# revdotcom/reverb

Measured on AMD Instinct MI355X. Metric: RTFx (audio-sec/wall-sec) Reverb-ASR attention_rescoring, higher is better.
Workload: dtype bf16

## Files before the change

reverb_amd/csrc/engine.h:

```cpp
#pragma once
#include <condition_variable>
#include <functional>
#include <map>
#include <mutex>
#include <string>
#include <thread>
#include <vector>

#include "../../include/rvb.h"
#include "kernels.h"
#include "search.h"

namespace rvb {

struct HostTensor {
  std::vector<float> data;
  std::vector<int64_t> shape;
  size_t numel() const { size_t n = 1; for (auto s : shape) n *= (size_t)s; return n; }
};

struct DevBuf {
  void* p = nullptr;
  size_t bytes = 0;
  int ensure(size_t n);
// ... 93 lines not shown
  unsigned long long gen_ = 0;
  bool stop_ = false;
};

struct HypRef { int chunk, idx, len, row0; };

struct TrieBatch {
  int R = 0, P = 0, max_chunk_rows = 0;
  std::vector<int32_t> tok, pos;
  std::vector<int32_t> path;
  std::vector<int32_t> hq_start, hq_len, hq_pos0, hkv_start, hkv_len;
  std::vector<int32_t> crow_start, crow_len;
  std::vector<int32_t> tgt_ptr, tgt;
  std::vector<int32_t> pair_slot;
  std::vector<int32_t> work;
};

struct CtcAligner {
  std::vector<VitSeq> seq;
  std::vector<int32_t> h_tokens, h_rows;
  int max_S = 0, blank = 0;
  size_t alpha_floats = 0, bp_bytes = 0;
  int64_t total_frames = 0;
  DevBuf d_tokens, d_rows, d_seqs, d_alpha, d_bp, d_states, d_score;
  int plan(const char* who, const int32_t* tokens, const int32_t* tok_lens, int n_seq, const std::vector<std::vector<int32_t>>& seq_rows,
           int V, int blank_id);
  int begin(hipStream_t s);
  bool touches(int r0, int nrows) const;
  int advance(hipStream_t s, const float* lp, int ld, int r0, int nrows);
  int finish(hipStream_t s, int32_t* states , float* score );
  void release();
};

}

struct rvb_engine {
  rvb_model_cfg cfg;
  int device = 0;
  int dtype = 0;
  bool fp8 = false;
  int f8_state = 0;
  std::vector<rvb::F8Scales> f8;
  std::vector<unsigned> f8_groups;
  rvb::DevBuf d_amax;
  bool f8_conv2 = false;
  float f8_x1 = 0.f;
  rvb::DevBuf d_f8sat;
  hipStream_t stream = nullptr;
  bool finalized = false;

  std::map<std::string, rvb::HostTensor> host;

  rvb::DevBuf cmvn_mean, cmvn_istd, conv1_w, conv1_b;
  rvb::Linear conv2, embed_out, ctc;
  rvb::LNorm enc_after;
  std::vector<rvb::EncLayer> enc;
  rvb::Decoder dec_l, dec_r;
  rvb::DevBuf pe_f32;
  int pe_rows = 0;
  rvb::DevBuf fb_window, fb_twiddle, fb_melw, fb_lo, fb_hi;
  rvb::DevBuf stage;

  rvb::DevBuf pcm, feats;
  rvb::DevBuf pcm_next;
  hipStream_t copy_stream = nullptr;
  hipEvent_t pcm_ready = nullptr, pcm_free = nullptr;
  bool pcm_pending = false;
  int64_t n_samples_next = 0;
  rvb::DevBuf wave_f32, rs_kernel;
  rvb::DevBuf wave_in;
  bool pcm_is_float = false;
  int dec_chunk = 0, dec_left = -1;
  int64_t n_samples = 0, n_frames = 0, feat_rows = 0;

  int B = 0, T0 = 0, T1 = 0, F1 = 0, T2 = 0, F2 = 0, beam = 0;
  std::vector<int32_t> in_lens, enc_lens;
  rvb::DevBuf d_feats_in, X1, X2, x, xn, y, h, ao, dconv, enc_out, logits, topv, topi;
  rvb::DevBuf d_enc_lens, d_seq_start, d_seq_len, d_aux_i32;
  float* h_topv = nullptr;
  int32_t* h_topi = nullptr;
  size_t h_top_cap = 0;
  struct Slice { int c0, nb; hipEvent_t ev; bool done; };
  std::vector<Slice> slices;
  std::vector<hipEvent_t> slice_event_pool;
  int xattn_max_rows = 0;
  const int* cur_lens = nullptr;
  std::vector<rvb::PrefixResult> nbest;
  std::vector<rvb::RescoreResult> rescored;
  std::vector<rvb::TrieBatch> trie_l;
  rvb::HostPool pool;
  std::vector<rvb::JointResult> joint;
  std::vector<rvb::DevBuf> jkv;
  rvb::DevBuf jlogp, jpair_row, jpair_tok, jpair_out;
  int64_t joint_rows = 0, joint_steps = 0;
  float last_blank_penalty = 0.f;
  std::vector<std::vector<int>> attn_tokens;
  std::vector<float> attn_scores;
  rvb::DevBuf atopv, atopi;
  std::vector<rvb::DevBuf> kcache, vcache, kcache2, vcache2, memkv;
  rvb::DevBuf dx, dxn, dy, dh, dqkv, dq, dao, kvmem, d_tok, d_pos, d_tgt, d_logp;
  rvb::DevBuf d_hq_start, d_hq_len, d_hkv_start, d_hkv_len;
  rvb::DevBuf d_hq_pos0, d_hpath_start, d_hpath_len, d_path, d_work, d_tgt_ptr;
  int64_t rescore_rows = 0, rescore_pairs = 0;

  struct StreamState {
    bool active = false;
    int offset = 0;
    int cache_len = 0;
    std::vector<rvb::DevBuf> kv, kv2;
    int cnn_rows = 0;
    std::vector<rvb::DevBuf> cnn, cnn2;
  } stream_st;
  rvb::DevBuf d_stream_i32;

  rvb::CtcAligner aligner;
  rvb::DevBuf align_lp, align_tv, align_ti, align_row, align_col, align_out;

  void* comm = nullptr;
  int comm_world = 1, comm_rank = 0;
  rvb::DevBuf comm_send, comm_recv;

  int profiling = 0;
  std::map<std::string, rvb::ProfEntry> prof;
  struct Pending { hipEvent_t a, b; std::string name; };
  std::vector<Pending> pending;
  std::vector<hipEvent_t> event_pool;
};
```

reverb_amd/csrc/engine.hip:

```cpp
#include "engine.h"

#include <algorithm>
#include <atomic>
#include <condition_variable>
#include <functional>
#include <mutex>
#include <chrono>
#include <cmath>
#include <cstdlib>
#include <cstring>
#include <thread>

namespace rvb {

static thread_local std::string g_err;
void set_error(const std::string& msg) { g_err = msg; }
const char* last_error() { return g_err.c_str(); }

int DevBuf::ensure(size_t n) {
  if (n <= bytes && p) return OK;
  if (p) { (void)hipFree(p); p = nullptr; bytes = 0; }
  if (n == 0) n = 16;
  hipError_t err = hipMalloc(&p, n);
  if (err != hipSuccess) {
    p = nullptr;
    (void)hipGetLastError();
    set_error("hipMalloc of " + std::to_string(n) + " bytes failed: " + hipGetErrorString(err));
    return E_NOMEM;
  }
  bytes = n;
  return OK;
}
void DevBuf::release() { if (p) (void)hipFree(p); p = nullptr; bytes = 0; }

#define RVB_TRY(expr) do { int _r = (expr); if (_r != OK) return _r; } while (0)

struct Scope {
  rvb_engine* e; hipEvent_t a = nullptr, b = nullptr; std::string name;
  Scope(rvb_engine* e_, const char* n, double flops = 0.0, double bytes = 0.0) : e(e_), name(n) {
    auto& pe = e->prof[name];
    pe.launches += 1; pe.flops += flops; pe.bytes += bytes;
    if (e->profiling == 0 || (e->profiling == 2 && name != "gemm" && name != "gemm_fp8")) return;
    auto get = [&]() { hipEvent_t ev; if (!e->event_pool.empty()) { ev = e->event_pool.back(); e->event_pool.pop_back(); } else (void)hipEventCreate(&ev); return ev; };
    a = get(); b = get();
    (void)hipEventRecord(a, e->stream);
  }
  ~Scope() {
    if (!a) return;
    (void)hipEventRecord(b, e->stream);
    e->pending.push_back({a, b, name});
  }
};
static void drain_prof(rvb_engine* e) {
  if (e->pending.empty()) return;
  (void)hipStreamSynchronize(e->stream);
  for (auto& p : e->pending) {
    float ms = 0.f;
    (void)hipEventElapsedTime(&ms, p.a, p.b);
    e->prof[p.name].ms += ms;
    e->event_pool.push_back(p.a); e->event_pool.push_back(p.b);
  }
  e->pending.clear();
}

static int upload_f32(rvb_engine* e, DevBuf& dst, const float* src, size_t n) {
  RVB_TRY(dst.ensure(n * 4));
  RVB_HIP_CHECK(hipMemcpyAsync(dst.p, src, n * 4, hipMemcpyHostToDevice, e->stream));
  return OK;
}
static int upload_i32(rvb_engine* e, DevBuf& dst, const int32_t* src, size_t n) {
  RVB_TRY(dst.ensure(n * 4 + 16));
  if (n) RVB_HIP_CHECK(hipMemcpyAsync(dst.p, src, n * 4, hipMemcpyHostToDevice, e->stream));
  return OK;
}
static int pack_T(rvb_engine* e, DevBuf& dst, const float* src, size_t n) {
  RVB_TRY(dst.ensure(n * dt_size(e->dtype)));
  if (e->dtype == DT_F32) {
    RVB_HIP_CHECK(hipMemcpyAsync(dst.p, src, n * 4, hipMemcpyHostToDevice, e->stream));
    return OK;
  }
  RVB_TRY(e->stage.ensure(n * 4));
  RVB_HIP_CHECK(hipMemcpyAsync(e->stage.p, src, n * 4, hipMemcpyHostToDevice, e->stream));
  return convert_f32(e->stream, e->dtype, e->stage.as<float>(), dst.p, n);
}
static int pack_linear(rvb_engine* e, Linear& L, const float* w, const float* b, int out, int in, bool f8 = false) {
  L.out = out; L.in = in;
  RVB_TRY(pack_T(e, L.w, w, (size_t)out * in));
  if (b) RVB_TRY(upload_f32(e, L.b, b, out)); else L.b.release();
  if (f8 && e->fp8 && in % 128 == 0) {
    std::vector<uint8_t> q((size_t)out * in);
    std::vector<float> sc(out);
    for (int n = 0; n < out; ++n) {
      const float* row = w + (size_t)n * in;
      float am = 0.f;
      for (int k = 0; k < in; ++k) am = std::max(am, std::fabs(row[k]));
      const float sn = am > 0.f ? am / 448.f : 1.f;
      sc[n] = sn;
      const float inv = 1.f / sn;
      for (int k = 0; k < in; ++k) q[(size_t)n * in + k] = f32_to_fp8_host(row[k] * inv);
    }
    RVB_TRY(L.w8.ensure(q.size()));
    RVB_HIP_CHECK(hipMemcpyAsync(L.w8.p, q.data(), q.size(), hipMemcpyHostToDevice, e->stream));
    RVB_TRY(upload_f32(e, L.wscale, sc.data(), out));
    RVB_HIP_CHECK(hipStreamSynchronize(e->stream));
  }
  return OK;
}

static const HostTensor* find(rvb_engine* e, const std::string& name) {
  auto it = e->host.find(name);
  return it == e->host.end() ? nullptr : &it->second;
}
static int need(rvb_engine* e, const std::string& name, size_t numel, const HostTensor** out) {
  const HostTensor* t = find(e, name);
  if (!t) { set_error("missing tensor: " + name); return E_STATE; }
  if (t->numel() != numel) {
    set_error("tensor " + name + " has " + std::to_string(t->numel()) + " elements, expected " + std::to_string(numel));
    return E_ARG;
  }
  *out = t;
  return OK;
}
static int pack_named_linear(rvb_engine* e, Linear& L, const std::string& p, int out, int in, bool bias = true, bool f8 = false) {
  const HostTensor *w, *b = nullptr;
  RVB_TRY(need(e, p + ".weight", (size_t)out * in, &w));
  if (bias) RVB_TRY(need(e, p + ".bias", out, &b));
  return pack_linear(e, L, w->data.data(), b ? b->data.data() : nullptr, out, in, f8);
}
static int pack_norm(rvb_engine* e, LNorm& n, const std::string& p, int d, float eps) {
  const HostTensor *g, *b;
  RVB_TRY(need(e, p + ".weight", d, &g));
  RVB_TRY(need(e, p + ".bias", d, &b));
  n.eps = eps;
  RVB_TRY(upload_f32(e, n.g, g->data.data(), d));
  return upload_f32(e, n.b, b->data.data(), d);
}
static int pack_concat(rvb_engine* e, Linear& L, const std::vector<std::string>& names, int out_each, int in, bool f8 = false) {
  std::vector<float> w((size_t)names.size() * out_each * in), b((size_t)names.size() * out_each);
  for (size_t i = 0; i < names.size(); ++i) {
    const HostTensor *tw, *tb;
    RVB_TRY(need(e, names[i] + ".weight", (size_t)out_each * in, &tw));
    RVB_TRY(need(e, names[i] + ".bias", out_each, &tb));
    memcpy(w.data() + i * (size_t)out_each * in, tw->data.data(), (size_t)out_each * in * 4);
    memcpy(b.data() + i * (size_t)out_each, tb->data.data(), (size_t)out_each * 4);
  }
  int r = pack_linear(e, L, w.data(), b.data(), (int)names.size() * out_each, in, f8);
// ... 423 lines not shown
    RVB_TRY(run_norm(e, x, L.n_conv, e->xn.p, false, M, d, NORM_LN, 0, nullptr, nullptr, nullptr, sc8.in_pw1, 0.f, false, satp(3)));
    RVB_TRY(run_gemm8(e, e->xn.p, d, L.pw1, e->h.p, 2 * d, M, sc8.in_pw1, 0));
  } else {
    RVB_TRY(run_norm(e, x, L.n_conv, e->xn.p, false, M, d));
    RVB_TRY(note(3, e->xn.p, (size_t)M * d));
    {
      const char* ge = lab_env("RVB_GLU_FUSE");
      const int glu_on = ge ? atoi(ge) : GLU_FUSE_DEFAULT;
      GemmArgs t;
      memset(&t, 0, sizeof(t));
      t.A = e->xn.p; t.W = L.pw1_glu.w.p; t.bias = L.pw1_glu.b.as<float>(); t.C = e->h.p; t.M = M; t.N = 2 * d; t.K = d; t.lda = d; t.ldw = d;
      t.ldc = d; t.alpha = 1.f; t.act = ACT_GLU;
      glu_fused = glu_on && li < 0 && L.pw1_glu.w.p != nullptr && !cal && gemm_glu_supported(e->dtype, t);
      if (glu_fused) {
        Scope sc(e, "gemm", 2.0 * M * (double)t.N * t.K, gemm_alg_bytes(e, t));
        RVB_TRY(gemm(e->stream, e->dtype, t));
      } else {
        RVB_TRY(run_gemm(e, e->xn.p, d, L.pw1, e->h.p, 2 * d, M, false));
      }
    }
  }
  {
    GluDwArgs g;
    g.gated = glu_fused ? 1 : 0;
    g.G = e->h.p; g.pw1_bias = L.pw1.b.as<float>(); g.dw_w = L.dw_w.as<float>(); g.dw_b = L.dw_b.as<float>();
    g.lens = e->cur_lens; g.out = e->dconv.as<float>(); g.B = B; g.T = T; g.d = d; g.K = e->cfg.cnn_kernel;
    g.causal = e->cfg.cnn_causal ? 1 : 0;
    g.out_bf16 = e->dtype == DT_BF16 ? 1 : 0;
    const int lorder = g.K - 1;
    const bool cached = li >= 0 && g.causal && lorder > 0;
    if (cached) { g.hist = e->stream_st.cnn[li].p; g.hist_rows = e->stream_st.cnn_rows; }
    {
      Scope sc(e, "glu_dwconv");
      RVB_TRY(glu_dwconv(e->stream, e->dtype, g));
    }
    if (cached) {
      auto& st = e->stream_st;
      const size_t es = dt_size(e->dtype), rb = (size_t)2 * d * es;
      if (M >= lorder) {
        RVB_HIP_CHECK(hipMemcpyAsync(st.cnn[li].p, (const char*)e->h.p + (size_t)(M - lorder) * rb, (size_t)lorder * rb,
                                     hipMemcpyDeviceToDevice, e->stream));
      } else {
        RVB_HIP_CHECK(hipMemcpyAsync(st.cnn2[li].p, (const char*)st.cnn[li].p + (size_t)M * rb, (size_t)(lorder - M) * rb,
                                     hipMemcpyDeviceToDevice, e->stream));
        RVB_HIP_CHECK(hipMemcpyAsync((char*)st.cnn2[li].p + (size_t)(lorder - M) * rb, e->h.p, (size_t)M * rb,
                                     hipMemcpyDeviceToDevice, e->stream));
        std::swap(st.cnn[li], st.cnn2[li]);
      }
    }
  }
  const int cmode = e->cfg.cnn_norm == 0 ? NORM_LN : NORM_AFFINE;
  const bool dw16 = e->dtype == DT_BF16;
  if (f8_pw2) {
    RVB_TRY(run_norm(e, e->dconv.as<float>(), L.n_cnn, e->xn.p, false, M, d, cmode, 1, nullptr, nullptr, nullptr, sc8.in_pw2, 0.f, dw16, satp(4)));
    RVB_TRY(run_gemm8(e, e->xn.p, d, L.pw2, x, d, M, sc8.in_pw2, 1, 1.f, 1.f, ACT_NONE, x, d));
  } else {
    RVB_TRY(run_norm(e, e->dconv.as<float>(), L.n_cnn, e->xn.p, false, M, d, cmode, 1, nullptr, nullptr, nullptr, 0.f, 0.f, dw16));
    RVB_TRY(note(4, e->xn.p, (size_t)M * d));
    RVB_TRY(run_gemm(e, e->xn.p, d, L.pw2, x, d, M, true, 1.f, ACT_NONE, x, d));
  }
  if (f8_ff) {
    RVB_TRY(run_norm(e, x, L.n_ff, e->xn.p, false, M, d, NORM_LN, 0, nullptr, nullptr, nullptr, sc8.in_ff1, 0.f, false, satp(5)));
    RVB_TRY(run_gemm8(e, e->xn.p, d, L.ff1, e->h.p, ff, M, sc8.in_ff1, 2, sc8.h_ff, 1.f, ACT_SILU, nullptr, 0, satp(6)));
    RVB_TRY(run_gemm8(e, e->h.p, ff, L.ff2, x, d, M, sc8.h_ff, 1, 1.f, 0.5f, ACT_NONE, x, d));
  } else {
    RVB_TRY(run_norm(e, x, L.n_ff, e->xn.p, false, M, d));
    const void* ffin = e->xn.p;
    if (L.is_lsl) {
      RVB_TRY(run_gemm(e, e->xn.p, d, L.lsl, e->y.p, d, M, false));
      ffin = e->y.p;
    } else {
      RVB_TRY(note(5, e->xn.p, (size_t)M * d));
    }
    RVB_TRY(run_gemm(e, ffin, d, L.ff1, e->h.p, ff, M, false, 1.f, ACT_SILU));
    if (!L.is_lsl) RVB_TRY(note(6, e->h.p, (size_t)M * ff));
    RVB_TRY(run_gemm(e, e->h.p, ff, L.ff2, x, d, M, true, 0.5f, ACT_NONE, x, d));
  }
  RVB_TRY(run_norm(e, x, L.n_final, x, true, M, d, NORM_LN, 0, L.is_lsl ? e->y.p : nullptr, &next, next_out, 0.f, f8 ? next8 : 0.f, false,
                   nullptr, (f8 && next8 > 0.f && e->d_f8sat.p) ? e->d_f8sat.as<unsigned>() + (size_t)(lidx + 1) * 8 : nullptr));
  return OK;
}

static const int LOGIT_SLAB = 8192;

static int wait_slices(rvb_engine* e, int i);

static int encode_impl(rvb_engine* e, const float* feats, int64_t first_chunk, const int32_t* lens, int B, int T0,
                       int beam, float blank_penalty) {
  const rvb_model_cfg& c = e->cfg;
  if (!e->finalized) { set_error("rvb_encode before rvb_finalize"); return E_STATE; }
  if (B <= 0 || B > c.max_chunks || T0 < 7 || T0 > c.chunk_frames) {
    set_error("rvb_encode: need 1 <= B <= max_chunks and 7 <= T0 <= chunk_frames"); return E_ARG;
  }
  if (beam < 1 || beam > 64 || beam > c.vocab) { set_error("rvb_encode: beam must be in [1,64]"); return E_ARG; }
  RVB_HIP_CHECK(hipSetDevice(e->device));
  RVB_TRY(wait_slices(e, -1));
  e->stream_st.active = false;
  const int d = c.d_model, F0 = c.input_dim, V = c.vocab;
  const int T1 = (T0 - 3) / 2 + 1, F1 = (F0 - 3) / 2 + 1, T2 = (T1 - 3) / 2 + 1, F2 = (F1 - 3) / 2 + 1;
  const int M = B * T2;
  const size_t es = dt_size(e->dtype);
  e->B = B; e->T0 = T0; e->T1 = T1; e->F1 = F1; e->T2 = T2; e->F2 = F2; e->beam = beam;
  e->dec_l.kv_ready = e->dec_r.kv_ready = false;
  e->last_blank_penalty = blank_penalty;
  e->in_lens.assign(lens, lens + B);
  e->enc_lens.resize(B);
  std::vector<int32_t> starts(B), qlens(B, T2);
  for (int b = 0; b < B; ++b) {
    if (lens[b] < 0 || lens[b] > T0) { set_error("rvb_encode: lens out of range"); return E_ARG; }
    e->enc_lens[b] = lens[b] > 6 ? (lens[b] - 7) / 4 + 1 : 0;
    starts[b] = b * T2;
  }
  e->nbest.clear(); e->trie_l.clear(); e->rescored.clear();
  RVB_TRY(upload_i32(e, e->d_enc_lens, e->enc_lens.data(), B));
  RVB_TRY(upload_i32(e, e->d_seq_start, starts.data(), B));
  RVB_TRY(upload_i32(e, e->d_seq_len, qlens.data(), B));

  const float* d_feats;
  if (feats) {
    RVB_TRY(upload_f32(e, e->d_feats_in, feats, (size_t)B * T0 * F0));
    d_feats = e->d_feats_in.as<float>();
  } else {
    if (!e->feats.p || (first_chunk + B) * (int64_t)T0 > e->feat_rows) {
      set_error("rvb_encode: device features missing or too short (call rvb_fbank first)"); return E_STATE;
    }
    d_feats = e->feats.as<float>() + (size_t)first_chunk * T0 * F0;
  }
  int SB = B >= 16 ? (B * 7 + 9) / 10 : B;
  if (B >= 64) SB = B - 32;
  if (const char* ov = lab_env("RVB_SLICE0")) { const int v = atoi(ov); if (v > 0 && v <= B) SB = v; }
  const int Ms = SB * T2;
  RVB_TRY(e->X1.ensure((size_t)SB * T1 * F1 * d * es));
  RVB_TRY(e->X2.ensure((size_t)SB * T2 * F2 * d * es));
  RVB_TRY(e->x.ensure((size_t)Ms * d * 4));
  RVB_TRY(e->xn.ensure((size_t)Ms * d * es));
  RVB_TRY(e->y.ensure((size_t)Ms * d * es));
  RVB_TRY(e->ao.ensure((size_t)Ms * d * es));
  RVB_TRY(e->dconv.ensure((size_t)Ms * d * 4));
  RVB_TRY(e->enc_out.ensure((size_t)M * d * es));
  RVB_TRY(e->h.ensure((size_t)Ms * std::max(c.ffn_dim, 3 * d) * es));
  const int Vld = (V + 3) & ~3;
  RVB_TRY(e->logits.ensure((size_t)LOGIT_SLAB * Vld * 4));
  RVB_TRY(e->topv.ensure((size_t)M * beam * 4));
  RVB_TRY(e->topi.ensure((size_t)M * beam * 4));
  if (e->h_top_cap < (size_t)M * beam) {
    if (e->h_topv) (void)hipHostFree(e->h_topv);
    if (e->h_topi) (void)hipHostFree(e->h_topi);
    e->h_topv = nullptr; e->h_topi = nullptr; e->h_top_cap = 0;
    RVB_HIP_CHECK(hipHostMalloc((void**)&e->h_topv, (size_t)M * beam * 4, hipHostMallocDefault));
    RVB_HIP_CHECK(hipHostMalloc((void**)&e->h_topi, (size_t)M * beam * 4, hipHostMallocDefault));
    e->h_top_cap = (size_t)M * beam;
  }
  e->slices.clear();
  if (e->fp8 && e->f8_state == 0) {
    RVB_TRY(e->d_amax.ensure((e->enc.size() + 1) * 8 * 4));
    RVB_HIP_CHECK(hipMemsetAsync(e->d_amax.p, 0, (e->enc.size() + 1) * 8 * 4, e->stream));
    RVB_TRY(reset_f8sat(e));
    e->f8_state = 1;
  }
  for (int c0 = 0; c0 < B; c0 += SB) {
    const int nb = std::min(SB, B - c0);
    const int m = nb * T2;
    const int row0 = c0 * T2;
    e->cur_lens = e->d_enc_lens.as<int>() + c0;
    const bool f8c2 = e->fp8 && e->f8_state == 2 && e->f8_conv2 && e->f8_x1 > 0.f && e->conv2.w8.p && d % 128 == 0;
    const bool calx = e->fp8 && e->f8_state == 1;
    {
      Scope sc(e, "subsample");
      RVB_TRY(subsample_conv1(e->stream, e->dtype, d_feats + (size_t)c0 * T0 * F0, e->cmvn_mean.as<float>(),
                              e->cmvn_istd.as<float>(), e->conv1_w.as<float>(), e->conv1_b.as<float>(), e->X1.p, nb, T0, F0, d,
                              f8c2 ? e->f8_x1 : 0.f, calx ? e->d_amax.as<unsigned>() + e->enc.size() * 8 : nullptr,
                              (f8c2 && e->d_f8sat.p) ? e->d_f8sat.as<unsigned>() + e->enc.size() * 8 + 1 : nullptr));
    }
    {
      GemmArgs g;
      memset(&g, 0, sizeof(g));
      g.A = e->X1.p; g.W = e->conv2.w.p; g.bias = e->conv2.b.as<float>(); g.C = e->X2.p;
      g.M = nb * T2 * F2; g.N = d; g.K = 9 * d; g.lda = d; g.ldw = 9 * d; g.ldc = d;
      g.alpha = 1.f; g.act = ACT_RELU; g.conv = 1; g.cT1 = T1; g.cF1 = F1; g.cT2 = T2; g.cF2 = F2; g.cC = d;
      if (f8c2) { g.W = e->conv2.w8.p; g.in_fp8 = 1; g.a_scale = e->f8_x1; g.w_scale = e->conv2.wscale.as<float>(); }
      Scope sc(e, f8c2 ? "gemm_fp8" : "gemm", 2.0 * g.M * (double)g.N * g.K, gemm_alg_bytes(e, g));
      RVB_TRY(gemm(e->stream, e->dtype, g));
    }
    RVB_TRY(run_gemm(e, e->X2.p, F2 * d, e->embed_out, e->x.p, d, m, true, std::sqrt((float)d)));
    void* eo = (char*)e->enc_out.p + (size_t)row0 * d * es;
    const bool f8 = e->fp8 && e->f8_state == 2;
    RVB_TRY(run_norm(e, e->x.as<float>(), e->enc[0].n_ffm, e->xn.p, false, m, d, NORM_LN, 0, nullptr, nullptr, nullptr,
                     (f8 && (e->f8_groups[0] & 1u)) ? e->f8[0].in_ffm1 : 0.f, 0.f, false, e->d_f8sat.as<unsigned>()));
    for (size_t li = 0; li < e->enc.size(); ++li) {
      const bool last = li + 1 == e->enc.size();
      RVB_TRY(encoder_layer(e, e->enc[li], (int)li, m, nb, T2, last ? e->enc_after : e->enc[li + 1].n_ffm, last ? eo : e->xn.p,
                            (f8 && !last && (e->f8_groups[li + 1] & 1u)) ? e->f8[li + 1].in_ffm1 : 0.f));
    }
    for (int r0 = 0; r0 < m; r0 += LOGIT_SLAB) {
      const int rows = std::min(LOGIT_SLAB, m - r0);
      RVB_TRY(run_gemm(e, (const char*)eo + (size_t)r0 * d * es, d, e->ctc, e->logits.p, Vld, rows, true));
      Scope sc(e, "ctc_topk");
      RVB_TRY(logsoftmax_topk(e->stream, e->logits.as<float>(), rows, V, Vld, beam, blank_penalty, c.blank_id,
                              e->topv.as<float>() + (size_t)(row0 + r0) * beam, e->topi.as<int>() + (size_t)(row0 + r0) * beam, nullptr));
    }
    RVB_HIP_CHECK(hipMemcpyAsync(e->h_topv + (size_t)row0 * beam, e->topv.as<float>() + (size_t)row0 * beam, (size_t)m * beam * 4, hipMemcpyDeviceToHost, e->stream));
    RVB_HIP_CHECK(hipMemcpyAsync(e->h_topi + (size_t)row0 * beam, e->topi.as<int>() + (size_t)row0 * beam, (size_t)m * beam * 4, hipMemcpyDeviceToHost, e->stream));
    hipEvent_t ev;
    if (!e->slice_event_pool.empty()) { ev = e->slice_event_pool.back(); e->slice_event_pool.pop_back(); }
    else RVB_HIP_CHECK(hipEventCreateWithFlags(&ev, hipEventDisableTiming));
    RVB_HIP_CHECK(hipEventRecord(ev, e->stream));
    e->slices.push_back({c0, nb, ev, false});
  }
  if (e->f8_state == 1) {
    std::vector<float> am((e->enc.size() + 1) * 8);
    RVB_HIP_CHECK(hipMemcpyAsync(am.data(), e->d_amax.p, am.size() * 4, hipMemcpyDeviceToHost, e->stream));
    RVB_HIP_CHECK(hipStreamSynchronize(e->stream));
    e->f8.resize(e->enc.size());
    auto sc = [](float a) { return a > 0.f ? std::exp2(std::ceil(std::log2(2.f * a / 448.f))) : 1.f; };
    for (size_t l = 0; l < e->enc.size(); ++l) {
      const float* a = am.data() + l * 8;
      e->f8[l] = {sc(a[0]), sc(a[1]), sc(a[2]), sc(a[3]), sc(a[4]), sc(a[5]), sc(a[6])};
    }
    e->f8_x1 = am[e->enc.size() * 8] > 0.f ? sc(am[e->enc.size() * 8]) : 0.f;
    if (e->f8_groups.size() != e->enc.size()) RVB_TRY(set_fp8_policy_impl(e, -1, 0, -1));
    e->f8_state = 2;
  }
  return OK;
}

static int wait_slices(rvb_engine* e, int i) {
  for (size_t k = 0; k < e->slices.size(); ++k) {
    if (i >= 0 && (int)k != i) continue;
    auto& sl = e->slices[k];
    if (sl.done) continue;
    RVB_HIP_CHECK(hipEventSynchronize(sl.ev));
    e->slice_event_pool.push_back(sl.ev);
    sl.done = true;
  }
  return OK;
}

static int stream_begin_impl(rvb_engine* e) {
  if (!e->finalized) { set_error("rvb_stream_begin before rvb_finalize"); return E_STATE; }
  RVB_HIP_CHECK(hipSetDevice(e->device));
  RVB_TRY(wait_slices(e, -1));
  const int d = e->cfg.d_model;
  const size_t es = dt_size(e->dtype);
  auto& st = e->stream_st;
  st.kv.resize(e->enc.size()); st.kv2.resize(e->enc.size());
  for (size_t l = 0; l < e->enc.size(); ++l) {
    RVB_TRY(st.kv[l].ensure((size_t)e->pe_rows * 2 * d * es));
    RVB_TRY(st.kv2[l].ensure((size_t)e->pe_rows * 2 * d * es));
  }
  RVB_TRY(e->enc_out.ensure((size_t)e->pe_rows * d * es));
  if (e->cfg.cnn_causal && e->cfg.cnn_kernel > 1) {
    st.cnn.resize(e->enc.size()); st.cnn2.resize(e->enc.size());
    for (size_t l = 0; l < e->enc.size(); ++l) {
      RVB_TRY(st.cnn[l].ensure((size_t)(e->cfg.cnn_kernel - 1) * 2 * d * es));
      RVB_TRY(st.cnn2[l].ensure((size_t)(e->cfg.cnn_kernel - 1) * 2 * d * es));
    }
  }
  st.active = true; st.offset = 0; st.cache_len = 0; st.cnn_rows = 0;
  e->B = 0; e->nbest.clear(); e->trie_l.clear(); e->rescored.clear(); e->slices.clear();
  e->dec_l.kv_ready = e->dec_r.kv_ready = false;
  return OK;
}

static int stream_chunk_impl(rvb_engine* e, const float* feats, int T0, int required_cache_size, float* out, int32_t* n_out) {
  const rvb_model_cfg& c = e->cfg;
  auto& st = e->stream_st;
  if (!st.active) { set_error("rvb_stream_chunk before rvb_stream_begin"); return E_STATE; }
  if (T0 < 7) { set_error("rvb_stream_chunk: a chunk needs at least 7 input frames (Conv2dSubsampling4)"); return E_ARG; }
  RVB_HIP_CHECK(hipSetDevice(e->device));
  const int d = c.d_model, F0 = c.input_dim;
  const int T1 = (T0 - 3) / 2 + 1, F1 = (F0 - 3) / 2 + 1, T2 = (T1 - 3) / 2 + 1, F2 = (F1 - 3) / 2 + 1;
  const int M = T2;
  const size_t es = dt_size(e->dtype);
  if (st.offset + M > e->pe_rows) {
    set_error("rvb_stream_chunk: more than " + std::to_string(e->pe_rows) + " encoder frames in one stream (the reference's positional "
              "table has max_len 5000 rows, embedding.py:33)");
    return E_UNSUPPORTED;
  }
  RVB_TRY(e->X1.ensure((size_t)T1 * F1 * d * es));
  RVB_TRY(e->X2.ensure((size_t)T2 * F2 * d * es));
  RVB_TRY(e->x.ensure((size_t)M * d * 4));
  RVB_TRY(e->xn.ensure((size_t)M * d * es));
  RVB_TRY(e->y.ensure((size_t)M * d * es));
  RVB_TRY(e->ao.ensure((size_t)M * d * es));
  RVB_TRY(e->dconv.ensure((size_t)M * d * 4));
  RVB_TRY(e->h.ensure((size_t)M * std::max(c.ffn_dim, 3 * d) * es));
  RVB_TRY(upload_f32(e, e->d_feats_in, feats, (size_t)T0 * F0));
  const int32_t zero = 0, mm = M, kv[2] = {0, st.cache_len + M};
  RVB_TRY(upload_i32(e, e->d_seq_start, &zero, 1));
  RVB_TRY(upload_i32(e, e->d_seq_len, &mm, 1));
  RVB_TRY(upload_i32(e, e->d_enc_lens, &mm, 1));
// ... 870 lines not shown
  for (int b = 0; b < B; ++b) js[b].result(&e->joint[b]);
  for (int b = 0; b < B; ++b)
    if (js[b].ties_cut() && K < V) {
      set_error("rvb_joint_decode: a frame of chunk " + std::to_string(b) + " has more than " + std::to_string(K - pre_beam) +
                " log-probs that tie exactly with the pre-beam threshold; keep more per frame (rvb_encode's beam argument, up to 64)");
      return E_UNSUPPORTED;
    }
  RVB_HIP_CHECK(hipStreamSynchronize(e->stream));
  return OK;
}

}

using namespace rvb;

extern "C" {

const char* rvb_last_error(void) { return last_error(); }
const char* rvb_version(void) { return "librvb 0.1 (gfx950)"; }

}
namespace rvb {
#ifdef RVB_TEST_API
const char* lab_env(const char* name) { return getenv(name); }
#else
const char* lab_env(const char*) { return nullptr; }
#endif
void attention_lab_switches(AttnArgs& a) {
  static const int sw[2] = {
      (lab_env("RVB_ATTN_OCC") && atoi(lab_env("RVB_ATTN_OCC")) == 3 ? ATTN_LAB_OCC3 : 0) |
          (lab_env("RVB_ATTN_MF") && atoi(lab_env("RVB_ATTN_MF")) == 0 ? ATTN_LAB_MF1 : 0) |
          (lab_env("RVB_ATTN_PADK") && atoi(lab_env("RVB_ATTN_PADK")) == 16 ? ATTN_LAB_PADK16 : 0),
      lab_env("RVB_ATTN_PLAIN") ? atoi(lab_env("RVB_ATTN_PLAIN")) : 0};
  a.lab |= sw[0];
  if (sw[1]) a.plain_order = 1;
}
}
extern "C" {

int rvb_model_cfg_size(void) { return (int)sizeof(rvb_model_cfg); }

int rvb_wer_counts(const int32_t* ref, int64_t n_ref, const int32_t* hyp, int64_t n_hyp, int64_t* counts) {
  if ((!ref && n_ref > 0) || (!hyp && n_hyp > 0) || !counts || n_ref < 0 || n_hyp < 0) { set_error("rvb_wer_counts: bad argument"); return E_ARG; }
  edit_counts(ref, n_ref, hyp, n_hyp, counts);
  return OK;
}

int rvb_create(const rvb_model_cfg* cfg, int device, rvb_engine** out) {
  if (!cfg || !out) { set_error("rvb_create: null argument"); return E_ARG; }
  if (cfg->struct_size != (int32_t)sizeof(rvb_model_cfg)) {
    set_error("rvb_create: ABI mismatch: rvb_model_cfg.struct_size is " + std::to_string(cfg->struct_size) + ", this library's struct has " +
              std::to_string(sizeof(rvb_model_cfg)) + " bytes (bind it field by field from include/rvb.h)");
    return E_ARG;
  }
  if (cfg->dtype != RVB_F32 && cfg->dtype != RVB_BF16 && cfg->dtype != RVB_FP8) { set_error("rvb_create: bad dtype"); return E_ARG; }
  if (cfg->d_model <= 0 || cfg->heads <= 0 || cfg->d_model % cfg->heads || cfg->d_model % 8 || cfg->ffn_dim % 8 ||
      cfg->dec_ffn_dim % 8 || cfg->input_dim != 80 || cfg->vocab < 2 || cfg->num_blocks < 1 ||
      cfg->cnn_kernel < 1 || cfg->cnn_kernel > 31 || (!cfg->cnn_causal && (cfg->cnn_kernel % 2) == 0) ||
      cfg->chunk_frames < 7 || cfg->max_chunks < 1 ||
      (cfg->dec_blocks > 0 && (cfg->dec_heads <= 0 || cfg->d_model % cfg->dec_heads))) {
    set_error("rvb_create: unsupported model dimensions (need d, ffn dims % 8 == 0, d % heads == 0, input_dim 80, cnn kernel <= 31 and odd unless causal)");
    return E_ARG;
  }
  int ndev = 0;
  hipError_t err = hipGetDeviceCount(&ndev);
  if (err != hipSuccess || ndev <= 0) { set_error("no HIP device available: librvb has no CPU fallback"); return E_HIP; }
  if (device < 0 || device >= ndev) { set_error("rvb_create: device index out of range"); return E_ARG; }
  RVB_HIP_CHECK(hipSetDevice(device));
  rvb_engine* e = new rvb_engine();
  e->cfg = *cfg; e->device = device;
  e->fp8 = cfg->dtype == RVB_FP8;
  e->dtype = e->fp8 ? (int)DT_BF16 : cfg->dtype;
  hipError_t se = hipStreamCreateWithFlags(&e->stream, hipStreamNonBlocking);
  if (se != hipSuccess) { delete e; set_error("hipStreamCreate failed"); return E_HIP; }
  *out = e;
  return OK;
}

void rvb_destroy(rvb_engine* e) {
  if (!e) return;
  (void)rvb_comm_destroy(e);
  (void)hipSetDevice(e->device);
  (void)hipStreamSynchronize(e->stream);
  DevBuf* bufs[] = {&e->cmvn_mean, &e->cmvn_istd, &e->conv1_w, &e->conv1_b, &e->pe_f32, &e->stage, &e->pcm, &e->feats,
                    &e->d_feats_in, &e->X1, &e->X2, &e->x, &e->xn, &e->y, &e->h, &e->ao, &e->dconv, &e->enc_out,
                    &e->logits, &e->topv, &e->topi, &e->d_enc_lens, &e->d_seq_start, &e->d_seq_len, &e->d_aux_i32,
                    &e->dx, &e->dxn, &e->dy, &e->dh, &e->dqkv, &e->dq, &e->dao, &e->kvmem, &e->d_tok, &e->d_pos,
                    &e->d_tgt, &e->d_logp, &e->d_hq_start, &e->d_hq_len, &e->d_hkv_start, &e->d_hkv_len,
                    &e->d_hq_pos0, &e->d_hpath_start, &e->d_hpath_len, &e->d_path, &e->d_work, &e->d_tgt_ptr,
                    &e->fb_window, &e->fb_twiddle, &e->fb_melw, &e->fb_lo, &e->fb_hi,
                    &e->conv2.w, &e->conv2.b, &e->embed_out.w, &e->embed_out.b, &e->ctc.w, &e->ctc.b,
                    &e->enc_after.g, &e->enc_after.b};
  for (DevBuf* b : bufs) b->release();
  e->aligner.release();
  for (DevBuf* b : {&e->align_lp, &e->align_tv, &e->align_ti, &e->align_row, &e->align_col, &e->align_out}) b->release();
  e->atopv.release(); e->atopi.release(); e->d_stream_i32.release(); e->d_amax.release(); e->d_f8sat.release();
  e->wave_f32.release(); e->wave_in.release(); e->rs_kernel.release();
  e->jlogp.release(); e->jpair_row.release(); e->jpair_tok.release(); e->jpair_out.release();
  for (auto& b : e->jkv) b.release();
  for (auto* v : {&e->stream_st.kv, &e->stream_st.kv2, &e->stream_st.cnn, &e->stream_st.cnn2}) for (auto& b : *v) b.release();
  for (auto* v : {&e->kcache, &e->vcache, &e->kcache2, &e->vcache2, &e->memkv}) for (auto& b : *v) b.release();
  auto rel_lin = [](Linear& l) { l.w.release(); l.b.release(); l.w8.release(); l.wscale.release(); };
  auto rel_n = [](LNorm& n) { n.g.release(); n.b.release(); };
  for (auto& L : e->enc) {
    for (Linear* l : {&L.ffm1, &L.ffm2, &L.ff1, &L.ff2, &L.qkv, &L.att_out, &L.pw1, &L.pw1_glu, &L.pw2, &L.lsl}) rel_lin(*l);
    for (LNorm* n : {&L.n_ffm, &L.n_mha, &L.n_conv, &L.n_ff, &L.n_final, &L.n_cnn}) rel_n(*n);
    L.pos_keys.release(); L.pos_bias.release(); L.bias_u.release(); L.bias_v.release(); L.dw_w.release(); L.dw_b.release();
  }
  for (Decoder* D : {&e->dec_l, &e->dec_r}) {
    D->embed.release(); rel_lin(D->out); rel_n(D->after);
    for (auto& L : D->layers) {
      for (Linear* l : {&L.self_qkv, &L.self_out, &L.src_q, &L.src_kv, &L.src_out, &L.ff1, &L.ff2, &L.lsl}) rel_lin(*l);
      for (LNorm* n : {&L.n1, &L.n2, &L.n3}) rel_n(*n);
      L.kvmem.release();
    }
  }
  if (e->h_topv) (void)hipHostFree(e->h_topv);
  if (e->h_topi) (void)hipHostFree(e->h_topi);
  for (auto& sl : e->slices) if (!sl.done) (void)hipEventDestroy(sl.ev);
  for (auto ev : e->slice_event_pool) (void)hipEventDestroy(ev);
  for (auto& p : e->pending) { (void)hipEventDestroy(p.a); (void)hipEventDestroy(p.b); }
  for (auto ev : e->event_pool) (void)hipEventDestroy(ev);
  if (e->copy_stream) (void)hipStreamDestroy(e->copy_stream);
  if (e->pcm_ready) (void)hipEventDestroy(e->pcm_ready);
  if (e->pcm_free) (void)hipEventDestroy(e->pcm_free);
  e->pcm_next.release();
  (void)hipStreamDestroy(e->stream);
  delete e;
}

int rvb_load_tensor(rvb_engine* e, const char* name, const float* host, const int64_t* shape, int ndim) {
  if (!e || !name || !host || ndim < 0 || (ndim > 0 && !shape)) { set_error("rvb_load_tensor: null argument"); return E_ARG; }
  HostTensor t;
  size_t n = 1;
  for (int i = 0; i < ndim; ++i) { if (shape[i] < 0) { set_error("negative dim"); return E_ARG; } t.shape.push_back(shape[i]); n *= (size_t)shape[i]; }
  t.data.assign(host, host + n);
  e->host[name] = std::move(t);
  return OK;
}

int rvb_finalize(rvb_engine* e, const float* cat_embs, int n_cat) {
  if (!e || (n_cat > 0 && !cat_embs)) { set_error("rvb_finalize: null argument"); return E_ARG; }
  return finalize_impl(e, cat_embs, n_cat);
}

int64_t rvb_num_frames(int64_t n) { return n < 400 ? 0 : 1 + (n - 400) / 160; }

static int drop_pending_upload(rvb_engine* e) {
  if (e->pcm_pending) {
    RVB_HIP_CHECK(hipStreamSynchronize(e->copy_stream));
    e->pcm_pending = false;
  }
  return OK;
}

int rvb_upload_pcm(rvb_engine* e, const int16_t* pcm, int64_t n) {
  if (!e || (!pcm && n > 0) || n < 0) { set_error("rvb_upload_pcm: bad argument"); return E_ARG; }
  RVB_HIP_CHECK(hipSetDevice(e->device));
  RVB_TRY(drop_pending_upload(e));
  RVB_TRY(e->pcm.ensure((size_t)n * 2 + 16));
  if (n) RVB_HIP_CHECK(hipMemcpyAsync(e->pcm.p, pcm, (size_t)n * 2, hipMemcpyHostToDevice, e->stream));
  RVB_HIP_CHECK(hipStreamSynchronize(e->stream));
  e->n_samples = n;
  e->pcm_is_float = false;
  return OK;
}

int rvb_upload_pcm_async(rvb_engine* e, const int16_t* pcm, int64_t n) {
  if (!e || (!pcm && n > 0) || n < 0) { set_error("rvb_upload_pcm_async: bad argument"); return E_ARG; }
  if (e->pcm_pending) { set_error("rvb_upload_pcm_async: an upload is already pending (consumed by the next rvb_fbank)"); return E_STATE; }
  RVB_HIP_CHECK(hipSetDevice(e->device));
  if (!e->copy_stream) {
    RVB_HIP_CHECK(hipStreamCreateWithFlags(&e->copy_stream, hipStreamNonBlocking));
    RVB_HIP_CHECK(hipEventCreateWithFlags(&e->pcm_ready, hipEventDisableTiming));
    RVB_HIP_CHECK(hipEventCreateWithFlags(&e->pcm_free, hipEventDisableTiming));
  }
  else RVB_HIP_CHECK(hipStreamWaitEvent(e->copy_stream, e->pcm_free, 0));
  RVB_TRY(e->pcm_next.ensure((size_t)n * 2 + 16));
  if (n) RVB_HIP_CHECK(hipMemcpyAsync(e->pcm_next.p, pcm, (size_t)n * 2, hipMemcpyHostToDevice, e->copy_stream));
  RVB_HIP_CHECK(hipEventRecord(e->pcm_ready, e->copy_stream));
  e->n_samples_next = n;
  e->pcm_pending = true;
  return OK;
}

int rvb_host_alloc(void** out, int64_t bytes) {
  if (!out || bytes < 0) { set_error("rvb_host_alloc: bad argument"); return E_ARG; }
  *out = nullptr;
  hipError_t err = hipHostMalloc(out, (size_t)std::max<int64_t>(bytes, 16), hipHostMallocDefault);
  if (err != hipSuccess) { *out = nullptr; set_error(std::string("hipHostMalloc: ") + hipGetErrorString(err)); return E_NOMEM; }
  return OK;
}
int rvb_host_free(void* p) {
  if (p) RVB_HIP_CHECK(hipHostFree(p));
  return OK;
}

int rvb_set_fp8_policy(rvb_engine* e, int groups, int first_block, int last_block) {
  if (!e) { set_error("rvb_set_fp8_policy: null engine"); return E_ARG; }
  if (!e->fp8) { set_error("rvb_set_fp8_policy: not an RVB_FP8 engine"); return E_STATE; }
  if (groups > 63 || first_block < 0) { set_error("rvb_set_fp8_policy: groups is a 6-bit mask (bit 5: the subsampling's conv2), first_block >= 0"); return E_ARG; }
  return set_fp8_policy_impl(e, groups, first_block, last_block);
}

int rvb_set_decoding_chunk(rvb_engine* e, int chunk_size, int num_left_chunks) {
// ... 616 lines not shown
```

Measured before the change: 28030.

## Run encoder batch slices concurrently on two HIP stream lanes

Splits the encoder batch into pairs of slices and runs them on two streams, each with its own workspace buffers, interleaving layer launches so the GPU can overlap kernels from both slices. The goal is to fill the device better when per-slice kernels underuse it and to hide the CTC/top-k tail. It also reworks profiling to merge overlapping spans across lanes. In exchange it uses extra workspace memory and cross-stream event synchronisation, and kernels on the two lanes may contend for the same compute units.

```diff
diff --git a/reverb_amd/csrc/engine.h b/reverb_amd/csrc/engine.h
--- a/reverb_amd/csrc/engine.h
+++ b/reverb_amd/csrc/engine.h
@@ -199,6 +199,13 @@
   size_t h_top_cap = 0;
   struct Slice { int c0, nb; hipEvent_t ev; bool done; };
   std::vector<Slice> slices;
+  struct Lane {
+    hipStream_t stream = nullptr;
+    rvb::DevBuf X1, X2, x, xn, y, ao, dconv, h, logits;
+    const int* cur_lens = nullptr;
+  } lane1;
+  int lane = 0;
+  hipEvent_t batch_ready = nullptr;
   std::vector<hipEvent_t> slice_event_pool;
   int xattn_max_rows = 0;
   const int* cur_lens = nullptr;
@@ -239,7 +246,8 @@
 
   int profiling = 0;
   std::map<std::string, rvb::ProfEntry> prof;
-  struct Pending { hipEvent_t a, b; std::string name; };
+  struct Pending { hipEvent_t a, b; std::string name; int lane; };
   std::vector<Pending> pending;
+  hipEvent_t prof_base = nullptr;
   std::vector<hipEvent_t> event_pool;
 };
diff --git a/reverb_amd/csrc/engine.hip b/reverb_amd/csrc/engine.hip
--- a/reverb_amd/csrc/engine.hip
+++ b/reverb_amd/csrc/engine.hip
@@ -35,33 +35,79 @@
 
 #define RVB_TRY(expr) do { int _r = (expr); if (_r != OK) return _r; } while (0)
 
+static hipEvent_t prof_event(rvb_engine* e) {
+  hipEvent_t ev;
+  if (!e->event_pool.empty()) { ev = e->event_pool.back(); e->event_pool.pop_back(); } else (void)hipEventCreate(&ev);
+  return ev;
+}
+static void prof_mark_base(rvb_engine* e) {
+  if (e->profiling == 0 || e->prof_base) return;
+  e->prof_base = prof_event(e);
+  (void)hipEventRecord(e->prof_base, e->stream);
+}
 struct Scope {
   rvb_engine* e; hipEvent_t a = nullptr, b = nullptr; std::string name;
   Scope(rvb_engine* e_, const char* n, double flops = 0.0, double bytes = 0.0) : e(e_), name(n) {
     auto& pe = e->prof[name];
     pe.launches += 1; pe.flops += flops; pe.bytes += bytes;
     if (e->profiling == 0 || (e->profiling == 2 && name != "gemm" && name != "gemm_fp8")) return;
-    auto get = [&]() { hipEvent_t ev; if (!e->event_pool.empty()) { ev = e->event_pool.back(); e->event_pool.pop_back(); } else (void)hipEventCreate(&ev); return ev; };
-    a = get(); b = get();
+    prof_mark_base(e);
+    a = prof_event(e); b = prof_event(e);
     (void)hipEventRecord(a, e->stream);
   }
   ~Scope() {
     if (!a) return;
     (void)hipEventRecord(b, e->stream);
-    e->pending.push_back({a, b, name});
+    e->pending.push_back({a, b, name, e->lane});
   }
 };
 static void drain_prof(rvb_engine* e) {
-  if (e->pending.empty()) return;
+  if (e->pending.empty()) {
+    if (e->prof_base) { e->event_pool.push_back(e->prof_base); e->prof_base = nullptr; }
+    return;
+  }
   (void)hipStreamSynchronize(e->stream);
+  if (e->lane1.stream) (void)hipStreamSynchronize(e->lane1.stream);
+  bool lanes = false;
+  for (auto& p : e->pending) lanes = lanes || p.lane != e->pending[0].lane;
+  std::map<std::string, std::vector<std::pair<double, double>>> spans;
   for (auto& p : e->pending) {
     float ms = 0.f;
     (void)hipEventElapsedTime(&ms, p.a, p.b);
-    e->prof[p.name].ms += ms;
+    if (!lanes) e->prof[p.name].ms += ms;
+    else {
+      float off = 0.f;
+      (void)hipEventElapsedTime(&off, e->prof_base, p.a);
+      spans[p.name].push_back({(double)off, (double)ms});
+    }
     e->event_pool.push_back(p.a); e->event_pool.push_back(p.b);
   }
+  for (auto& kv : spans) {
+    std::sort(kv.second.begin(), kv.second.end());
+    double total = 0.0, end = -1e300;
+    for (auto& [start, len] : kv.second) {
+      if (start >= end) total += len;
+      else if (start + len > end) total += start + len - end;
+      end = std::max(end, start + len);
+    }
+    e->prof[kv.first].ms += total;
+  }
   e->pending.clear();
-}
+  if (e->prof_base) { e->event_pool.push_back(e->prof_base); e->prof_base = nullptr; }
+}
+
+static void swap_lane(rvb_engine* e) {
+  auto& l = e->lane1;
+  std::swap(e->stream, l.stream); std::swap(e->cur_lens, l.cur_lens);
+  std::swap(e->X1, l.X1); std::swap(e->X2, l.X2); std::swap(e->x, l.x); std::swap(e->xn, l.xn); std::swap(e->y, l.y);
+  std::swap(e->ao, l.ao); std::swap(e->dconv, l.dconv); std::swap(e->h, l.h); std::swap(e->logits, l.logits);
+  e->lane ^= 1;
+}
+static void use_lane(rvb_engine* e, int k) { if (e->lane != k) swap_lane(e); }
+struct LaneGuard {
+  rvb_engine* e;
+  ~LaneGuard() { use_lane(e, 0); }
+};
 
 static int upload_f32(rvb_engine* e, DevBuf& dst, const float* src, size_t n) {
   RVB_TRY(dst.ensure(n * 4));
@@ -651,6 +697,8 @@
 }
 
 static const int LOGIT_SLAB = 8192;
+static constexpr int LANES_DEFAULT = 2;
+static constexpr int LANES_MIN_B = 64;
 
 static int wait_slices(rvb_engine* e, int i);
 
@@ -695,21 +743,49 @@
     }
     d_feats = e->feats.as<float>() + (size_t)first_chunk * T0 * F0;
   }
-  int SB = B >= 16 ? (B * 7 + 9) / 10 : B;
-  if (B >= 64) SB = B - 32;
-  if (const char* ov = lab_env("RVB_SLICE0")) { const int v = atoi(ov); if (v > 0 && v <= B) SB = v; }
-  const int Ms = SB * T2;
-  RVB_TRY(e->X1.ensure((size_t)SB * T1 * F1 * d * es));
-  RVB_TRY(e->X2.ensure((size_t)SB * T2 * F2 * d * es));
-  RVB_TRY(e->x.ensure((size_t)Ms * d * 4));
-  RVB_TRY(e->xn.ensure((size_t)Ms * d * es));
-  RVB_TRY(e->y.ensure((size_t)Ms * d * es));
-  RVB_TRY(e->ao.ensure((size_t)Ms * d * es));
-  RVB_TRY(e->dconv.ensure((size_t)Ms * d * 4));
+  std::vector<int> plan;
+  int lanes = (B >= LANES_MIN_B && LANES_DEFAULT == 2) ? 2 : 1;
+  if (const char* lv = lab_env("RVB_LANES")) { const int v = atoi(lv); if (v == 1 || (v == 2 && B >= 2)) lanes = v; }
+  if (e->fp8 && e->f8_state == 0) lanes = 1;
+  if (lanes == 1) {
+    int SB = B >= 16 ? (B * 7 + 9) / 10 : B;
+    if (B >= 64) SB = B - 32;
+    if (const char* ov = lab_env("RVB_SLICE0")) { const int v = atoi(ov); if (v > 0 && v <= B) SB = v; }
+    plan.push_back(SB);
+    if (B > SB) plan.push_back(B - SB);
+  } else {
+    const int tail = B >= 64 ? 32 : 0, body = B - tail;
+    plan = {(body + 1) / 2, body / 2};
+    if (tail) { plan.push_back(tail / 2); plan.push_back(tail / 2); }
+    if (const char* ov = lab_env("RVB_LANE_SPLIT")) {
+      std::vector<int> v;
+      int sum = 0;
+      for (const char* q = ov; *q;) { char* end; const long n = strtol(q, &end, 10); if (end == q || n <= 0) { sum = -1; break; } v.push_back((int)n); sum += (int)n; q = *end == ',' ? end + 1 : end; if (*end && *end != ',') { sum = -1; break; } }
+      if (sum == B && v.size() >= 2) plan = v;
+    }
+  }
+  const int Vld = (V + 3) & ~3;
+  auto ensure_ws = [&](int SB) -> int {
+    const int Ms = SB * T2;
+    RVB_TRY(e->X1.ensure((size_t)SB * T1 * F1 * d * es));
+    RVB_TRY(e->X2.ensure((size_t)SB * T2 * F2 * d * es));
+    RVB_TRY(e->x.ensure((size_t)Ms * d * 4));
+    RVB_TRY(e->xn.ensure((size_t)Ms * d * es));
+    RVB_TRY(e->y.ensure((size_t)Ms * d * es));
+    RVB_TRY(e->ao.ensure((size_t)Ms * d * es));
+    RVB_TRY(e->dconv.ensure((size_t)Ms * d * 4));
+    RVB_TRY(e->h.ensure((size_t)Ms * std::max(c.ffn_dim, 3 * d) * es));
+    return e->logits.ensure((size_t)LOGIT_SLAB * Vld * 4);
+  };
+  LaneGuard guard{e};
+  for (int k = 0; k < lanes; ++k) {
+    int most = 0;
+    for (size_t i = k; i < plan.size(); i += lanes) most = std::max(most, plan[i]);
+    use_lane(e, k);
+    RVB_TRY(ensure_ws(most));
+  }
+  use_lane(e, 0);
   RVB_TRY(e->enc_out.ensure((size_t)M * d * es));
-  RVB_TRY(e->h.ensure((size_t)Ms * std::max(c.ffn_dim, 3 * d) * es));
-  const int Vld = (V + 3) & ~3;
-  RVB_TRY(e->logits.ensure((size_t)LOGIT_SLAB * Vld * 4));
   RVB_TRY(e->topv.ensure((size_t)M * beam * 4));
   RVB_TRY(e->topi.ensure((size_t)M * beam * 4));
   if (e->h_top_cap < (size_t)M * beam) {
@@ -727,10 +803,17 @@
     RVB_TRY(reset_f8sat(e));
     e->f8_state = 1;
   }
-  for (int c0 = 0; c0 < B; c0 += SB) {
-    const int nb = std::min(SB, B - c0);
-    const int m = nb * T2;
-    const int row0 = c0 * T2;
+  if (lanes == 2) {
+    if (!e->lane1.stream) RVB_HIP_CHECK(hipStreamCreateWithFlags(&e->lane1.stream, hipStreamNonBlocking));
+    if (!e->batch_ready) RVB_HIP_CHECK(hipEventCreateWithFlags(&e->batch_ready, hipEventDisableTiming));
+    prof_mark_base(e);
+    RVB_HIP_CHECK(hipEventRecord(e->batch_ready, e->stream));
+    RVB_HIP_CHECK(hipStreamWaitEvent(e->lane1.stream, e->batch_ready, 0));
+  }
+  const bool f8 = e->fp8 && e->f8_state == 2;
+  struct Job { int c0, nb; };
+  auto front = [&](const Job& j) -> int {
+    const int c0 = j.c0, nb = j.nb, m = nb * T2;
     e->cur_lens = e->d_enc_lens.as<int>() + c0;
     const bool f8c2 = e->fp8 && e->f8_state == 2 && e->f8_conv2 && e->f8_x1 > 0.f && e->conv2.w8.p && d % 128 == 0;
     const bool calx = e->fp8 && e->f8_state == 1;
@@ -752,15 +835,18 @@
       RVB_TRY(gemm(e->stream, e->dtype, g));
     }
     RVB_TRY(run_gemm(e, e->X2.p, F2 * d, e->embed_out, e->x.p, d, m, true, std::sqrt((float)d)));
-    void* eo = (char*)e->enc_out.p + (size_t)row0 * d * es;
-    const bool f8 = e->fp8 && e->f8_state == 2;
-    RVB_TRY(run_norm(e, e->x.as<float>(), e->enc[0].n_ffm, e->xn.p, false, m, d, NORM_LN, 0, nullptr, nullptr, nullptr,
-                     (f8 && (e->f8_groups[0] & 1u)) ? e->f8[0].in_ffm1 : 0.f, 0.f, false, e->d_f8sat.as<unsigned>()));
-    for (size_t li = 0; li < e->enc.size(); ++li) {
-      const bool last = li + 1 == e->enc.size();
-      RVB_TRY(encoder_layer(e, e->enc[li], (int)li, m, nb, T2, last ? e->enc_after : e->enc[li + 1].n_ffm, last ? eo : e->xn.p,
-                            (f8 && !last && (e->f8_groups[li + 1] & 1u)) ? e->f8[li + 1].in_ffm1 : 0.f));
-    }
+    return run_norm(e, e->x.as<float>(), e->enc[0].n_ffm, e->xn.p, false, m, d, NORM_LN, 0, nullptr, nullptr, nullptr,
+                    (f8 && (e->f8_groups[0] & 1u)) ? e->f8[0].in_ffm1 : 0.f, 0.f, false, e->d_f8sat.as<unsigned>());
+  };
+  auto block = [&](const Job& j, size_t li) -> int {
+    void* eo = (char*)e->enc_out.p + (size_t)j.c0 * T2 * d * es;
+    const bool last = li + 1 == e->enc.size();
+    return encoder_layer(e, e->enc[li], (int)li, j.nb * T2, j.nb, T2, last ? e->enc_after : e->enc[li + 1].n_ffm, last ? eo : e->xn.p,
+                         (f8 && !last && (e->f8_groups[li + 1] & 1u)) ? e->f8[li + 1].in_ffm1 : 0.f);
+  };
+  auto back = [&](const Job& j) -> int {
+    const int m = j.nb * T2, row0 = j.c0 * T2;
+    const void* eo = (const char*)e->enc_out.p + (size_t)row0 * d * es;
     for (int r0 = 0; r0 < m; r0 += LOGIT_SLAB) {
       const int rows = std::min(LOGIT_SLAB, m - r0);
       RVB_TRY(run_gemm(e, (const char*)eo + (size_t)r0 * d * es, d, e->ctc, e->logits.p, Vld, rows, true));
@@ -774,8 +860,22 @@
     if (!e->slice_event_pool.empty()) { ev = e->slice_event_pool.back(); e->slice_event_pool.pop_back(); }
     else RVB_HIP_CHECK(hipEventCreateWithFlags(&ev, hipEventDisableTiming));
     RVB_HIP_CHECK(hipEventRecord(ev, e->stream));
-    e->slices.push_back({c0, nb, ev, false});
-  }
+    e->slices.push_back({j.c0, j.nb, ev, false});
+    return OK;
+  };
+  for (size_t i0 = 0, c0 = 0; i0 < plan.size(); i0 += lanes) {
+    Job jobs[2];
+    int n = 0;
+    for (; n < lanes && i0 + n < plan.size(); ++n) { jobs[n] = {(int)c0, plan[i0 + n]}; c0 += plan[i0 + n]; }
+    for (int k = 0; k < n; ++k) { use_lane(e, k); RVB_TRY(front(jobs[k])); }
+    for (size_t li = 0; li < e->enc.size(); ++li)
+      for (int k = 0; k < n; ++k) { use_lane(e, k); RVB_TRY(block(jobs[k], li)); }
+    for (int k = 0; k < n; ++k) { use_lane(e, k); RVB_TRY(back(jobs[k])); }
+  }
+  use_lane(e, 0);
+  if (lanes == 2)
+    for (size_t i = e->slices.size(); i-- > 0;)
+      if ((i % 2) == 1) { RVB_HIP_CHECK(hipStreamWaitEvent(e->stream, e->slices[i].ev, 0)); break; }
   if (e->f8_state == 1) {
     std::vector<float> am((e->enc.size() + 1) * 8);
     RVB_HIP_CHECK(hipMemcpyAsync(am.data(), e->d_amax.p, am.size() * 4, hipMemcpyDeviceToHost, e->stream));
@@ -1812,6 +1912,7 @@
   (void)rvb_comm_destroy(e);
   (void)hipSetDevice(e->device);
   (void)hipStreamSynchronize(e->stream);
+  if (e->lane1.stream) (void)hipStreamSynchronize(e->lane1.stream);
   DevBuf* bufs[] = {&e->cmvn_mean, &e->cmvn_istd, &e->conv1_w, &e->conv1_b, &e->pe_f32, &e->stage, &e->pcm, &e->feats,
                     &e->d_feats_in, &e->X1, &e->X2, &e->x, &e->xn, &e->y, &e->h, &e->ao, &e->dconv, &e->enc_out,
                     &e->logits, &e->topv, &e->topi, &e->d_enc_lens, &e->d_seq_start, &e->d_seq_len, &e->d_aux_i32,
@@ -1851,6 +1952,10 @@
   for (auto ev : e->slice_event_pool) (void)hipEventDestroy(ev);
   for (auto& p : e->pending) { (void)hipEventDestroy(p.a); (void)hipEventDestroy(p.b); }
   for (auto ev : e->event_pool) (void)hipEventDestroy(ev);
+  if (e->prof_base) (void)hipEventDestroy(e->prof_base);
+  { auto& l = e->lane1; for (DevBuf* b : {&l.X1, &l.X2, &l.x, &l.xn, &l.y, &l.ao, &l.dconv, &l.h, &l.logits}) b->release(); }
+  if (e->batch_ready) (void)hipEventDestroy(e->batch_ready);
+  if (e->lane1.stream) (void)hipStreamDestroy(e->lane1.stream);
   if (e->copy_stream) (void)hipStreamDestroy(e->copy_stream);
   if (e->pcm_ready) (void)hipEventDestroy(e->pcm_ready);
   if (e->pcm_free) (void)hipEventDestroy(e->pcm_free);
```

After: 28070, median of 2. No clear change (+0.2%).
